# pdh930105/ARCQuant

Measured on AMD Instinct MI355X. Metric: ARC-NVFP4 GEMM TFLOP/s (M=4096, N=KQ=4096, KE=64), higher is better.
Workload: dtype f16

## Files before the change

### arcquant_amd/csrc/gemm_tile.hip

```cpp
#include <hip/hip_runtime.h>
#include <stdint.h>
#include <stdlib.h>

#include <type_traits>

#include "arcq_internal.hpp"
#include "gemm_common.hpp"
#include "gemm_tile_common.hpp"

namespace arcq {

#ifdef ARCQ_STREAM_STAMPS
static unsigned long long* g_tile_stamps = nullptr;
#ifndef ARCQ_TILE_REPACKED_UNIT
extern "C" void arcq_debug_set_tile_stamps(void* p) { g_tile_stamps = reinterpret_cast<unsigned long long*>(p); }
#endif
#define ARCQ_TILE_STAMP(k)                                                                                     \
  do {                                                                                                         \
    if (p.stamps && tid == 0) {                                                                                \
      unsigned long long t0_, t1_;                                                                             \
      asm volatile("s_memtime %0\n\ts_memrealtime %1\n\ts_waitcnt lgkmcnt(0)" : "=s"(t0_), "=s"(t1_)::"memory"); \
      p.stamps[(size_t)blockIdx.x * (2 * kTileStamps) + 2 * (k)] = t0_;                                        \
      p.stamps[(size_t)blockIdx.x * (2 * kTileStamps) + 2 * (k) + 1] = t1_;                                    \
    }                                                                                                          \
  } while (0)
#else
#define ARCQ_TILE_STAMP(k) do { } while (0)
#endif

#ifndef ARCQ_TILE_WIDE_STORES
#define ARCQ_TILE_WIDE_STORES 1
#endif

template <int BM, int BN, int WAVES_M, int WAVES_N, bool kMfma32, int kEpi, bool kStagger, bool kPipe, int kBLayout = kBRef>
__global__ __launch_bounds__(WAVES_M* WAVES_N * 64) void gemm_tile_kernel(TileParams p) {
  constexpr int kThreads = WAVES_M * WAVES_N * 64;
  constexpr int WM = BM / WAVES_M, WN = BN / WAVES_N;
  constexpr int kT = kMfma32 ? 32 : 16;
  constexpr int TM = WM / kT, TN = WN / kT;
  using acc_t = typename std::conditional<kMfma32, f32x16, f32x4>::type;
  constexpr int A_UNITS = (BM * 2 + kThreads - 1) / kThreads, B_UNITS = (BN * 2 + kThreads - 1) / kThreads;
  constexpr bool A_PARTIAL = (BM * 2) % kThreads != 0, B_PARTIAL = (BN * 2) % kThreads != 0;
  static_assert(!A_PARTIAL || A_UNITS == 1, "a partial A pass is a single pass");
  static_assert(!B_PARTIAL || B_UNITS == 1, "a partial B pass is a single pass");
  constexpr int A_TILE = BM * kRowBytes, B_TILE = BN * kRowBytes;

  extern __shared__ __attribute__((aligned(16))) unsigned char smem[];
  unsigned char* const lds_a0 = smem;
  unsigned char* const lds_b0 = smem + A_TILE;
  unsigned char* const lds_a1 = smem + A_TILE + B_TILE;
  unsigned char* const lds_b1 = smem + 2 * A_TILE + B_TILE;

  const int ntiles = p.tiles_m * p.tiles_n;
  int bid = blockIdx.x, split = 0;
  if (p.splits > 1) {
    split = bid / ntiles;
    bid -= split * ntiles;
  }
  {
    const int q8 = ntiles >> 3, r8 = ntiles & 7, x = bid & 7, j = bid >> 3;
    bid = (x < r8 ? x * (q8 + 1) : r8 * (q8 + 1) + (x - r8) * q8) + j;
  }
  constexpr int kGroupM = 8;
  const int per_group = kGroupM * p.tiles_n;
  const int grp = bid / per_group;
  const int first_m = grp * kGroupM;
  const int gsz = min(p.tiles_m - first_m, kGroupM);
  const int tm = first_m + (bid % per_group) % gsz;
  const int tn = (bid % per_group) / gsz;
  const int m0 = __builtin_amdgcn_readfirstlane(tm * BM), n0 = __builtin_amdgcn_readfirstlane(tn * BN);

  const int tid = threadIdx.x;
  const int lane = tid & 63, wave = tid >> 6;
  const int wr = wave / WAVES_N, wc = wave % WAVES_N;
  ARCQ_TILE_STAMP(0);
  const int half_k = p.K >> 1, atoms_k = p.K >> 6;
  const int a_begin = split * p.atoms_per_split, a_end = min(atoms_k, a_begin + p.atoms_per_split);

  const uint8_t* a_q[A_UNITS];
  const uint8_t* a_sf[A_UNITS];
  uint32_t a_live[A_UNITS];
  int a_slot[A_UNITS][4];
#pragma unroll
  for (int u = 0; u < A_UNITS; ++u) {
    const int unit = tid + u * kThreads, r = A_PARTIAL ? min(unit >> 1, BM - 1) : unit >> 1, h = unit & 1;
    const int row = m0 + r, rc = row < p.M ? row : p.M - 1;
    a_q[u] = p.A + (size_t)rc * half_k + h * 16;
    a_sf[u] = p.SFA + sf_atom_offset(rc, 0, atoms_k) + h * 2;
    a_live[u] = row < p.M ? 0xffffu : 0u;
#pragma unroll
    for (int j = 0; j < 4; ++j) a_slot[u][j] = kMfma32 ? lds_slot32(r, h * 4 + j) : lds_slot(r, h * 4 + j);
  }
  const uint8_t* b_q[B_UNITS];
  const uint8_t* b_sf[B_UNITS];
  uint32_t b_live[B_UNITS];
  int b_slot[B_UNITS][4];
#pragma unroll
  for (int u = 0; u < B_UNITS; ++u) {
    const int unit = tid + u * kThreads, r = B_PARTIAL ? min(unit >> 1, BN - 1) : unit >> 1, h = unit & 1;
    const int row = n0 + r, rc = row < p.N ? row : p.N - 1;
    if constexpr (kBLayout == kBRepacked) {
      const int tiles = ((p.K + 255) >> 8) * 2;
      b_q[u] = p.B + (size_t)(rc >> 4) * tiles * 1024 + h * 256 + (rc & 15) * 16;
      b_sf[u] = p.SFB + (size_t)(rc >> 4) * tiles * 128 + h * 64 + (rc & 15) * 4;
    } else {
      b_q[u] = p.B + (size_t)rc * half_k + h * 16;
      b_sf[u] = p.SFB + sf_atom_offset(rc, 0, atoms_k) + h * 2;
    }
    b_live[u] = row < p.N ? 0xffffu : 0u;
#pragma unroll
    for (int j = 0; j < 4; ++j) b_slot[u][j] = kMfma32 ? lds_slot32(r, h * 4 + j) : lds_slot(r, h * 4 + j);
  }
  const int fa_base = kMfma32 ? lds_slot32(wr * WM + (lane & 31), lane >> 5) : lds_slot(wr * WM + (lane & 15), lane >> 4);
  const int fb_base = kMfma32 ? lds_slot32(wc * WN + (lane & 31), lane >> 5) : lds_slot(wc * WN + (lane & 15), lane >> 4);
  acc_t acc[TM][TN];
#pragma unroll
  for (int i = 0; i < TM; ++i)
#pragma unroll
    for (int j = 0; j < TN; ++j)
#pragma unroll
      for (int r = 0; r < (kMfma32 ? 16 : 4); ++r) acc[i][j][r] = 0.f;

  Staged sa[A_UNITS], sb[B_UNITS];
  auto load_step = [&](int atom) {
#pragma unroll
    for (int u = 0; u < A_UNITS; ++u) sa[u] = stage_load(a_q[u], a_sf[u], atom);
#pragma unroll
    for (int u = 0; u < B_UNITS; ++u) sb[u] = kBLayout == kBRepacked ? stage_load_rw(b_q[u], b_sf[u], atom) : stage_load(b_q[u], b_sf[u], atom);
  };
  auto store_step = [&](unsigned char* la, unsigned char* lb) {
#pragma unroll
    for (int u = 0; u < A_UNITS; ++u)
      if (!A_PARTIAL || tid < BM * 2) stage_store(la, a_slot[u], sa[u], a_live[u]);
#pragma unroll
    for (int u = 0; u < B_UNITS; ++u)
      if (!B_PARTIAL || tid < BN * 2) stage_store(lb, b_slot[u], sb[u], b_live[u]);
  };
  auto mma_step = [&](const unsigned char* la, const unsigned char* lb) {
    if constexpr (kMfma32) {
#pragma unroll
      for (int ks = 0; ks < 4; ++ks) {
        Frag8 fa[TM], fb[TN];
#pragma unroll
        for (int i = 0; i < TM; ++i) fa[i].u = *reinterpret_cast<const uint4*>(la + (fa_base ^ (ks * 32)) + i * 32 * kRowBytes);
#pragma unroll
        for (int j = 0; j < TN; ++j) fb[j].u = *reinterpret_cast<const uint4*>(lb + (fb_base ^ (ks * 32)) + j * 32 * kRowBytes);
#pragma unroll
        for (int i = 0; i < TM; ++i)
#pragma unroll
          for (int j = 0; j < TN; ++j) acc[i][j] = __builtin_amdgcn_mfma_f32_32x32x16_f16(fb[j].v, fa[i].v, acc[i][j], 0, 0, 0);
      }
    } else {
#pragma unroll
      for (int ks = 0; ks < 2; ++ks) {
        Frag8 fa[TM], fb[TN];
#pragma unroll
        for (int i = 0; i < TM; ++i) fa[i].u = *reinterpret_cast<const uint4*>(la + (fa_base ^ (ks * 64)) + i * 16 * kRowBytes);
#pragma unroll
        for (int j = 0; j < TN; ++j) fb[j].u = *reinterpret_cast<const uint4*>(lb + (fb_base ^ (ks * 64)) + j * 16 * kRowBytes);
#pragma unroll
        for (int i = 0; i < TM; ++i)
#pragma unroll
          for (int j = 0; j < TN; ++j) acc[i][j] = __builtin_amdgcn_mfma_f32_16x16x32_f16(fb[j].v, fa[i].v, acc[i][j], 0, 0, 0);
      }
    }
  };
  const bool late = kStagger && wave >= 4;
  auto k_step = [&](int kt, unsigned char* ca, unsigned char* cb, unsigned char* na, unsigned char* nb) {
    Staged ta[A_UNITS], tb[B_UNITS];
#pragma unroll
    for (int u = 0; u < A_UNITS; ++u) ta[u] = sa[u];
#pragma unroll
    for (int u = 0; u < B_UNITS; ++u) tb[u] = sb[u];
    load_step(min(kt + 2 + (late ? 1 : 0), a_end - 1));
    __builtin_amdgcn_sched_barrier(0);
    mma_step(ca, cb);
    if (kStagger && late) __syncthreads();
    unsigned char* const wa = late ? ca : na;
    unsigned char* const wb = late ? cb : nb;
#pragma unroll
    for (int u = 0; u < A_UNITS; ++u)
      if (!A_PARTIAL || tid < BM * 2) stage_store(wa, a_slot[u], ta[u], a_live[u]);
#pragma unroll
    for (int u = 0; u < B_UNITS; ++u)
      if (!B_PARTIAL || tid < BN * 2) stage_store(wb, b_slot[u], tb[u], b_live[u]);
    if (!kStagger || !late) __syncthreads();
  };

  auto k_step_pipe = [&](int kt, unsigned char* ca, unsigned char* cb, unsigned char* na, unsigned char* nb) {
    static_assert(kMfma32 || TM % 2 == 0, "pairs of A fragments");
    Staged ta[A_UNITS], tb[B_UNITS];
#pragma unroll
    for (int u = 0; u < A_UNITS; ++u) ta[u] = sa[u];
#pragma unroll
    for (int u = 0; u < B_UNITS; ++u) tb[u] = sb[u];
    load_step(min(kt + 2, a_end - 1));
    __builtin_amdgcn_sched_barrier(0);
    constexpr int kPieces = (A_UNITS + B_UNITS) * 4, kBlocks = kMfma32 ? 4 : TM;
    auto pieces = [&](int blk) {
#pragma unroll
      for (int c = blk; c < kPieces; c += kBlocks) {
        const int u = c >> 2, j = c & 3;
        if (u < A_UNITS) {
#ifdef ARCQ_EXPERIMENT_A_RAW
          if (!A_PARTIAL || tid < BM * 2) stage_piece_raw(na, a_slot[u < A_UNITS ? u : 0][j], ta[u < A_UNITS ? u : 0], a_live[u < A_UNITS ? u : 0], j);
#else
          if (!A_PARTIAL || tid < BM * 2) stage_piece(na, a_slot[u < A_UNITS ? u : 0][j], ta[u < A_UNITS ? u : 0], a_live[u < A_UNITS ? u : 0], j);
#endif
        } else {
          const int v = u - A_UNITS < B_UNITS ? u - A_UNITS : 0;
#ifdef ARCQ_EXPERIMENT_B_RAW
          if (!B_PARTIAL || tid < BN * 2) stage_piece_raw(nb, b_slot[v][j], tb[v], b_live[v], j);
#else
          if (!B_PARTIAL || tid < BN * 2) stage_piece(nb, b_slot[v][j], tb[v], b_live[v], j);
#endif
        }
      }
    };
    if constexpr (kMfma32) {
      Frag8 f32a[2][TM], f32b[2][TN];
      auto rd_set = [&](int buf, int ks) {
#pragma unroll
        for (int i = 0; i < TM; ++i) f32a[buf][i].u = *reinterpret_cast<const uint4*>(ca + (fa_base ^ (ks * 32)) + i * 32 * kRowBytes);
#pragma unroll
        for (int j = 0; j < TN; ++j) f32b[buf][j].u = *reinterpret_cast<const uint4*>(cb + (fb_base ^ (ks * 32)) + j * 32 * kRowBytes);
      };
      rd_set(0, 0);
#pragma unroll
      for (int ks = 0; ks < 4; ++ks) {
        if (ks + 1 < 4) rd_set((ks + 1) & 1, ks + 1);
        __builtin_amdgcn_sched_barrier(0);
#pragma unroll
        for (int i = 0; i < TM; ++i)
#pragma unroll
          for (int j = 0; j < TN; ++j)
            if constexpr (kMfma32)
              acc[i][j] = __builtin_amdgcn_mfma_f32_32x32x16_f16(f32b[ks & 1][j].v, f32a[ks & 1][i].v, acc[i][j], 0, 0, 0);
        pieces(ks);
        __builtin_amdgcn_sched_barrier(0);
      }
      __syncthreads();
      return;
    }
    auto rd_a = [&](int ks, int i) { Frag8 f; f.u = *reinterpret_cast<const uint4*>(ca + (fa_base ^ (ks * 64)) + i * 16 * kRowBytes); return f; };
    auto rd_b = [&](int ks, int j) { Frag8 f; f.u = *reinterpret_cast<const uint4*>(cb + (fb_base ^ (ks * 64)) + j * 16 * kRowBytes); return f; };
    constexpr int kPairs = TM / 2, kSeq = 2 * kPairs, kAhead = 1;
    Frag8 fb[2][TN], fq[kSeq][2];
    auto rd_pair = [&](int q) {
      fq[q][0] = rd_a(q / kPairs, 2 * (q % kPairs));
      fq[q][1] = rd_a(q / kPairs, 2 * (q % kPairs) + 1);
    };
#pragma unroll
    for (int j = 0; j < TN; ++j) fb[0][j] = rd_b(0, j);
#pragma unroll
    for (int q = 0; q < kAhead; ++q) rd_pair(q);
#pragma unroll
    for (int q = 0; q < kSeq; ++q) {
      const int ks = q / kPairs, pr = q % kPairs;
      if (q + kAhead < kSeq) rd_pair(q + kAhead);
      if (ks == 0 && pr == kPairs - 1 - (kAhead - 1 < kPairs - 1 ? kAhead - 1 : kPairs - 1)) {
#pragma unroll
        for (int j = 0; j < TN; ++j) fb[1][j] = rd_b(1, j);
      }
      __builtin_amdgcn_sched_barrier(0);
#pragma unroll
      for (int ii = 0; ii < 2; ++ii)
#pragma unroll
        for (int j = 0; j < TN; ++j)
          if constexpr (!kMfma32)
            acc[2 * pr + ii][j] = __builtin_amdgcn_mfma_f32_16x16x32_f16(fb[ks][j].v, fq[q][ii].v, acc[2 * pr + ii][j], 0, 0, 0);
      pieces(q);
#pragma unroll
      for (int m8 = 0; m8 < (TM == 8 ? 2 * TN : 0); ++m8) {
        __builtin_amdgcn_sched_group_barrier(0x008, 1, 0);
        __builtin_amdgcn_sched_group_barrier(0x002, 2, 0);
      }
      __builtin_amdgcn_sched_barrier(0);
    }
    __syncthreads();
  };

  load_step(a_begin);
  Staged sa0[A_UNITS], sb0[B_UNITS];
#pragma unroll
  for (int u = 0; u < A_UNITS; ++u) sa0[u] = sa[u];
#pragma unroll
  for (int u = 0; u < B_UNITS; ++u) sb0[u] = sb[u];
  load_step(min(a_begin + 1, a_end - 1));
  __builtin_amdgcn_sched_barrier(0);
#pragma unroll
  for (int u = 0; u < A_UNITS; ++u)
    if (!A_PARTIAL || tid < BM * 2) stage_store(lds_a0, a_slot[u], sa0[u], a_live[u]);
#pragma unroll
  for (int u = 0; u < B_UNITS; ++u)
    if (!B_PARTIAL || tid < BN * 2) stage_store(lds_b0, b_slot[u], sb0[u], b_live[u]);
  if (kStagger && late) {
    store_step(lds_a1, lds_b1);
    load_step(min(a_begin + 2, a_end - 1));
  }
  __syncthreads();
  int kt = a_begin;
#ifndef ARCQ_EXPERIMENT_GENERAL_EPILOGUE
  float alpha_dev = 1.0f;
  if (p.alpha_dev) alpha_dev = *reinterpret_cast<const __attribute__((address_space(4))) float*>(reinterpret_cast<uintptr_t>(p.alpha_dev));
  asm volatile("" : "+s"(alpha_dev));
#endif
  if (WAVES_M * WAVES_N == 8 && wave >= 4) __builtin_amdgcn_s_setprio(1);
  ARCQ_TILE_STAMP(1);
  if constexpr (kPipe) {
    for (; kt + 1 < a_end; kt += 2) {
      k_step_pipe(kt, lds_a0, lds_b0, lds_a1, lds_b1);
      k_step_pipe(kt + 1, lds_a1, lds_b1, lds_a0, lds_b0);
    }
    if (kt < a_end) k_step_pipe(kt, lds_a0, lds_b0, lds_a1, lds_b1);
  } else {
    for (; kt + 1 < a_end; kt += 2) {
      k_step(kt, lds_a0, lds_b0, lds_a1, lds_b1);
      k_step(kt + 1, lds_a1, lds_b1, lds_a0, lds_b0);
    }
    if (kt < a_end) k_step(kt, lds_a0, lds_b0, lds_a1, lds_b1);
  }
  ARCQ_TILE_STAMP(2);

#ifdef ARCQ_EXPERIMENT_GENERAL_EPILOGUE
  const float alpha = p.alpha_host * (p.alpha_dev ? *p.alpha_dev : 1.0f);
#else
  const float alpha = p.alpha_host * alpha_dev;
#endif
  const bool vec_ok = (p.N & 3) == 0;
  uint32_t act_max = 0;
  [[maybe_unused]] auto interior_epilogue = [&](auto has_bias, auto has_res) __attribute__((always_inline)) {
    constexpr bool kBias = decltype(has_bias)::value, kRes = decltype(has_res)::value;
    constexpr bool kSilu = kEpi == kEpiSiluMul;
    constexpr uint32_t kElem = kSilu ? 1 : 2;
    unsigned char* const tile_d = reinterpret_cast<unsigned char*>(p.D) + ((size_t)m0 * p.N + n0) * kElem;
    const unsigned char* const tile_r = kRes ? reinterpret_cast<const unsigned char*>(p.residual) + ((size_t)m0 * p.N + n0) * 2 : nullptr;
    uint32_t t = tid;
    asm volatile("" : "+v"(t));
    const uint32_t lane_row = (t >> 6) / WAVES_N * WM + (t & 15), lane_col = (t >> 6) % WAVES_N * WN + 4 * ((t >> 4) & 3);
    uint32_t off = lane_row * (uint32_t)p.N + lane_col;
    const uint32_t row_step = 16u * (uint32_t)p.N;
    constexpr bool kWide = ARCQ_TILE_WIDE_STORES && !kSilu && TN % 2 == 0;
    typedef uint32_t u32x4_a8 __attribute__((ext_vector_type(4), aligned(8)));
    [[maybe_unused]] const uint32_t g4 = (t >> 4) & 3;
    [[maybe_unused]] uint32_t off_w = off - 4 * g4 + ((g4 & 1) ? 16 + 4 * (g4 - 1) : 4 * g4);
    [[maybe_unused]] uint2 held = make_uint2(0, 0);
    float bias_f[TN][4];
    if constexpr (kBias) {
#pragma unroll
      for (int j = 0; j < TN; ++j) {
        const uint2 b = *reinterpret_cast<const uint2*>(p.bias + n0 + lane_col + j * 16);
        bias_f[j][0] = bf16_bits_to_f32(b.x & 0xffffu); bias_f[j][1] = bf16_bits_to_f32(b.x >> 16);
        bias_f[j][2] = bf16_bits_to_f32(b.y & 0xffffu); bias_f[j][3] = bf16_bits_to_f32(b.y >> 16);
      }
    }
    uint2 res_cur[TN], res_nxt[TN];
    auto res_load = [&](uint32_t o, uint2 (&r)[TN]) {
#pragma unroll
      for (int j = 0; j < TN; ++j) r[j] = *reinterpret_cast<const uint2*>(tile_r + (size_t)o * 2 + j * 32);
    };
    if constexpr (kRes) res_load(off, res_cur);
#pragma unroll
    for (int i = 0; i < TM; ++i) {
      if constexpr (kRes) { if (i + 1 < TM) res_load(off + row_step, res_nxt); }
#pragma unroll
      for (int j = 0; j < TN; ++j) {
        float d[4] = {alpha * acc[i][j][0], alpha * acc[i][j][1], alpha * acc[i][j][2], alpha * acc[i][j][3]};
        if constexpr (kSilu) {
          if constexpr (kBias) {
#pragma unroll
            for (int r = 0; r < 4; r += 2) {
              round2_to_bf16(d[r], d[r + 1]);
              d[r] += bias_f[j][r];
              d[r + 1] += bias_f[j][r + 1];
            }
          }
          const uint32_t y01 = pack_bf16x2_hw(d[0], d[1]), y23 = pack_bf16x2_hw(d[2], d[3]);
          const uint32_t a0 = silu_mul_bf16(y01 & 0xffffu, y01 >> 16), a1 = silu_mul_bf16(y23 & 0xffffu, y23 >> 16);
          *reinterpret_cast<uint32_t*>(tile_d + (size_t)off + j * 16) = a0 | (a1 << 16);
          act_max = max(act_max, max(a0 & 0x7fffu, a1 & 0x7fffu));
        } else {
          if constexpr (kBias) {
#pragma unroll
            for (int r = 0; r < 4; r += 2) {
              round2_to_bf16(d[r], d[r + 1]);
              d[r] += bias_f[j][r];
              d[r + 1] += bias_f[j][r + 1];
            }
          }
          if constexpr (kRes) {
            const uint32_t rw[2] = {res_cur[j].x, res_cur[j].y};
#pragma unroll
            for (int r = 0; r < 4; r += 2) {
              round2_to_bf16(d[r], d[r + 1]);
              d[r] += bf16_bits_to_f32(rw[r >> 1] & 0xffffu);
              d[r + 1] += bf16_bits_to_f32(rw[r >> 1] >> 16);
            }
          }
          const uint2 pk = make_uint2(pack_bf16x2_hw(d[0], d[1]), pack_bf16x2_hw(d[2], d[3]));
          if constexpr (kWide) {
            if (j & 1) {
              const auto lo = __builtin_amdgcn_permlane16_swap(held.x, pk.x, false, false);
              const auto hi = __builtin_amdgcn_permlane16_swap(held.y, pk.y, false, false);
              const u32x4_a8 v = {lo[0], hi[0], lo[1], hi[1]};
              *reinterpret_cast<u32x4_a8*>(tile_d + (size_t)off_w * 2 + (j >> 1) * 64) = v;
            } else {
              held = pk;
            }
          } else {
            *reinterpret_cast<uint2*>(tile_d + (size_t)off * 2 + j * 32) = pk;
          }
        }
        if (i == 0 && j == 0) ARCQ_TILE_STAMP(3);
      }
      if constexpr (kRes) {
#pragma unroll
        for (int j = 0; j < TN; ++j) res_cur[j] = res_nxt[j];
      }
      off += row_step;
      off_w += row_step;
    }
  };
  auto store4 = [&](int m, int n, float d0, float d1, float d2, float d3, bool pre, uint2 bias2, uint2 res2) __attribute__((always_inline)) {
    if (m >= p.M || n >= p.N) return;
    const uint32_t bw[2] = {bias2.x, bias2.y}, rw[2] = {res2.x, res2.y};
    auto bias_at = [&](int r) { return bf16_bits_to_f32(pre ? (bw[r >> 1] >> (16 * (r & 1))) & 0xffffu : (uint32_t)p.bias[n + r]); };
    if (kEpi == kEpiSiluMul) {
      uint32_t y[4] = {f32_to_bf16_bits(alpha * d0), f32_to_bf16_bits(alpha * d1), f32_to_bf16_bits(alpha * d2), f32_to_bf16_bits(alpha * d3)};
      if (p.bias) {
#pragma unroll
        for (int e = 0; e < 4; ++e) y[e] = f32_to_bf16_bits(bf16_bits_to_f32(y[e]) + bias_at(e));
      }
      const uint32_t a0 = silu_mul_bf16(y[0], y[1]);
      const uint32_t a1 = silu_mul_bf16(y[2], y[3]);
      *reinterpret_cast<uint32_t*>(reinterpret_cast<uint16_t*>(p.D) + (size_t)m * (p.N >> 1) + (n >> 1)) = a0 | (a1 << 16);
      act_max = max(act_max, max(a0 & 0x7fffu, a1 & 0x7fffu));
      return;
    }
    if (p.splits > 1) {
      *reinterpret_cast<float4*>(p.partial + ((size_t)split * p.M + m) * p.N + n) = make_float4(d0, d1, d2, d3);
      return;
    }
    float d[4] = {alpha * d0, alpha * d1, alpha * d2, alpha * d3};
    if (p.bias) {
#pragma unroll
      for (int r = 0; r < 4; ++r)
        if (pre || n + r < p.N) d[r] = (p.out_dtype == ARCQ_OUT_F32 ? d[r] : bf16_bits_to_f32(f32_to_bf16_bits(d[r]))) + bias_at(r);
    }
    if (p.residual) {
#pragma unroll
      for (int r = 0; r < 4; ++r)
        if (pre || n + r < p.N) {
          const float res = bf16_bits_to_f32(pre ? (rw[r >> 1] >> (16 * (r & 1))) & 0xffffu : (uint32_t)p.residual[(size_t)m * p.N + n + r]);
          d[r] = (p.out_dtype == ARCQ_OUT_F32 ? d[r] : bf16_bits_to_f32(f32_to_bf16_bits(d[r]))) + res;
        }
    }
    if (p.out_dtype == ARCQ_OUT_F32) {
      float* o = reinterpret_cast<float*>(p.D) + (size_t)m * p.N + n;
      if (vec_ok) *reinterpret_cast<float4*>(o) = make_float4(d[0], d[1], d[2], d[3]);
      else for (int r = 0; r < 4; ++r) if (n + r < p.N) o[r] = d[r];
    } else {
      uint16_t* o = reinterpret_cast<uint16_t*>(p.D) + (size_t)m * p.N + n;
      if (vec_ok) *reinterpret_cast<uint2*>(o) = make_uint2(pack_bf16x2(d[0], d[1]), pack_bf16x2(d[2], d[3]));
      else for (int r = 0; r < 4; ++r) if (n + r < p.N) o[r] = (uint16_t)f32_to_bf16_bits(d[r]);
    }
  };
#ifdef ARCQ_EXPERIMENT_GENERAL_EPILOGUE
  constexpr bool kInteriorPath = false;
#else
  constexpr bool kInteriorPath = !kMfma32;
#endif
  bool interior = false;
  if constexpr (kInteriorPath)
    interior = m0 + BM <= p.M && n0 + BN <= p.N && vec_ok && p.splits <= 1 && p.out_dtype == ARCQ_OUT_BF16 && (int64_t)BM * p.N < (1ll << 31) &&
               ((reinterpret_cast<uintptr_t>(p.bias) | reinterpret_cast<uintptr_t>(p.residual)) & 7) == 0;
  if (interior) {
    if constexpr (kInteriorPath) {
      using T = std::true_type;
      using F = std::false_type;
      if constexpr (kEpi == kEpiSiluMul) {
        if (p.bias) interior_epilogue(T{}, F{});
        else interior_epilogue(F{}, F{});
      } else if (p.bias) {
        if (p.residual) interior_epilogue(T{}, T{});
        else interior_epilogue(T{}, F{});
      } else {
        if (p.residual) interior_epilogue(F{}, T{});
        else interior_epilogue(F{}, F{});
      }
    }
  } else if constexpr (kMfma32) {
#pragma unroll
    for (int i = 0; i < TM; ++i)
#pragma unroll
      for (int j = 0; j < TN; ++j) {
        const int m = m0 + wr * WM + i * 32 + (lane & 31);
#pragma unroll
        for (int g = 0; g < 4; ++g) {
          const int n = n0 + wc * WN + j * 32 + 8 * g + 4 * (lane >> 5);
          store4(m, n, acc[i][j][4 * g + 0], acc[i][j][4 * g + 1], acc[i][j][4 * g + 2], acc[i][j][4 * g + 3], false, make_uint2(0, 0), make_uint2(0, 0));
        }
      }
  } else {
    const bool pre = vec_ok && p.splits <= 1 && ((reinterpret_cast<uintptr_t>(p.bias) | reinterpret_cast<uintptr_t>(p.residual)) & 7) == 0;
    const int nb = n0 + wc * WN + 4 * (lane >> 4), mb = m0 + wr * WM + (lane & 15);
    if (pre) {
      uint2 bias_v[TN], res_cur[TN], res_nxt[TN];
#pragma unroll
      for (int j = 0; j < TN; ++j) {
        bias_v[j] = res_cur[j] = res_nxt[j] = make_uint2(0, 0);
        if (p.bias && nb + j * 16 < p.N) bias_v[j] = *reinterpret_cast<const uint2*>(p.bias + nb + j * 16);
      }
      auto res_load = [&](int i, uint2 (&r)[TN]) {
        if (!p.residual) return;
        const int m = mb + i * 16;
#pragma unroll
        for (int j = 0; j < TN; ++j)
          if (m < p.M && nb + j * 16 < p.N) r[j] = *reinterpret_cast<const uint2*>(p.residual + (size_t)m * p.N + nb + j * 16);
      };
      res_load(0, res_cur);
#pragma unroll
      for (int i = 0; i < TM; ++i) {
        if (i + 1 < TM) res_load(i + 1, res_nxt);
#pragma unroll
        for (int j = 0; j < TN; ++j) {
          store4(mb + i * 16, nb + j * 16, acc[i][j][0], acc[i][j][1], acc[i][j][2], acc[i][j][3], true, bias_v[j], res_cur[j]);
          if (i == 0 && j == 0) ARCQ_TILE_STAMP(3);
        }
#pragma unroll
        for (int j = 0; j < TN; ++j) res_cur[j] = res_nxt[j];
      }
    } else {
#pragma unroll
      for (int i = 0; i < TM; ++i)
#pragma unroll
        for (int j = 0; j < TN; ++j) {
          store4(mb + i * 16, nb + j * 16, acc[i][j][0], acc[i][j][1], acc[i][j][2], acc[i][j][3], false, make_uint2(0, 0), make_uint2(0, 0));
          if (i == 0 && j == 0) ARCQ_TILE_STAMP(3);
        }
    }
  }
  ARCQ_TILE_STAMP(4);
  if (kEpi == kEpiSiluMul) {
    __shared__ uint32_t wave_max[WAVES_M * WAVES_N];
#pragma unroll
    for (int sh = 32; sh > 0; sh >>= 1) act_max = max(act_max, (uint32_t)__shfl_down((int)act_max, sh, 64));
    if (lane == 0) wave_max[wave] = act_max;
    __syncthreads();
    if (tid == 0) {
      uint32_t m = 0;
#pragma unroll
      for (int w = 0; w < WAVES_M * WAVES_N; ++w) m = max(m, wave_max[w]);
      p.slots[blockIdx.x] = m;
    }
  }
}

struct TileCfg { int id, bm, bn, waves; };
static constexpr TileCfg kTileCfgs[] = {{1, 128, 128, 4}, {2, 256, 256, 4}, {3, 256, 256, 8}, {4, 128, 256, 4}, {5, 256, 256, 8}, {6, 128, 128, 4},
                                        {7, 64, 256, 4}, {8, 32, 256, 4}, {9, 128, 128, 4}, {10, 128, 256, 8}, {11, 256, 128, 8}, {12, 128, 128, 8},
                                        {13, 64, 256, 8}, {14, 64, 128, 8}, {15, 64, 64, 4}, {16, 64, 128, 4}, {17, 128, 64, 4}};
static const TileCfg& tile_cfg(int id) {
  for (const TileCfg& c : kTileCfgs)
    if (c.id == id) return c;
  return kTileCfgs[2];
}

static int env_int(const char* name, int dflt) {
  const char* e = getenv(name);
  return e ? atoi(e) : dflt;
}
static int tile_cfg_override() {
  static const int v = env_int("ARCQ_TILE_CFG", 0);
  return v;
}
static int tile_split_override() {
  static const int v = env_int("ARCQ_TILE_SPLIT", 0);
  return v;
}
static bool tile_stagger() {
  static const int v = env_int("ARCQ_TILE_STAGGER", 0);
  return v != 0;
}
static bool tile_pipe() {
  static const int v = env_int("ARCQ_TILE_PIPE", 1);
  return v != 0;
}

static void tile_split(int64_t M, int64_t N, int64_t K, int BM, int BN, int* splits, int* atoms_per_split) {
  const int64_t tiles = ((M + BM - 1) / BM) * ((N + BN - 1) / BN);
  const int atoms = (int)(K / 64);
  int s = 1;
  if ((N % 4) == 0) {
    if (tile_split_override() > 0) s = min(tile_split_override(), max(atoms / 2, 1));
    else
      while (tiles * s < 256 && atoms / (s * 2) >= 8 && s < 32) s *= 2;
  }
  const int per = (atoms + s - 1) / s;
  *splits = (atoms + per - 1) / per;
  *atoms_per_split = per;
}

template <int BM, int BN, int WAVES_M, int WAVES_N, bool kMfma32 = false, int kEpi = kEpiPlain, int kBLayout = kBRef>
static int launch_tile(const GemmArgs& a, hipStream_t stream, bool allow_split = false) {
  TileParams p;
  p.A = a.A; p.B = a.B; p.SFA = a.SFA; p.SFB = a.SFB; p.D = a.D;
  p.alpha_dev = a.alpha_dev; p.bias = a.bias; p.residual = a.residual;
  p.M = a.M; p.N = a.N; p.K = a.K; p.alpha_host = a.alpha_host; p.out_dtype = a.out_dtype;
  p.tiles_m = (a.M + BM - 1) / BM;
  p.tiles_n = (a.N + BN - 1) / BN;
  p.splits = 1; p.atoms_per_split = a.K / 64; p.partial = nullptr;
  p.epi = a.epilogue; p.slots = a.absmax_slots;
#ifdef ARCQ_STREAM_STAMPS
  p.stamps = g_tile_stamps;
#endif
  if (allow_split && a.epilogue == kEpiPlain) {
    tile_split(a.M, a.N, a.K, BM, BN, &p.splits, &p.atoms_per_split);
    if (p.splits > 1) {
      const int64_t need = (int64_t)p.splits * a.M * a.N * (int64_t)sizeof(float);
      if (!a.workspace || a.workspace_bytes < need)
        return fail(ARCQ_ERR_WORKSPACE, "arcq_gemm_nvfp4: split-K needs %lld B of workspace, got %lld", (long long)need,
                    (long long)a.workspace_bytes);
      p.partial = reinterpret_cast<float*>(a.workspace);
    }
  }
  const size_t lds = 2 * (size_t)(BM + BN) * kRowBytes;
  constexpr bool kCanStagger = WAVES_M * WAVES_N == 8 && BM == 256 && BN == 256, kCanPipe = true;
  auto kern = gemm_tile_kernel<BM, BN, WAVES_M, WAVES_N, kMfma32, kEpi, false, false, kBLayout>;
  if (kCanPipe && tile_pipe()) kern = gemm_tile_kernel<BM, BN, WAVES_M, WAVES_N, kMfma32, kEpi, false, kCanPipe, kBLayout>;
  else if (kCanStagger && tile_stagger()) kern = gemm_tile_kernel<BM, BN, WAVES_M, WAVES_N, kMfma32, kEpi, kCanStagger, false, kBLayout>;
  static LdsOptIn lds_opt[3];
  const int which = (kCanPipe && tile_pipe()) ? 1 : (kCanStagger && tile_stagger()) ? 2 : 0;
  if (int rc = ensure_dynamic_lds(reinterpret_cast<const void*>(kern), lds_opt[which], (int)lds, "arcq_gemm_nvfp4 (tile)")) return rc;
  hipLaunchKernelGGL(kern, dim3((unsigned)(p.tiles_m * p.tiles_n * p.splits)), dim3(WAVES_M * WAVES_N * 64), lds, stream, p);
  hipError_t e = hipGetLastError();
  if (e != hipSuccess) return fail(ARCQ_ERR_LAUNCH, "arcq_gemm_nvfp4 (tile): launch failed: %s", hipGetErrorString(e));
  if (p.splits > 1) return gemm_splitk_finish(a, p.splits, stream);
  return ARCQ_OK;
}

static int tile_choice(int64_t M, int64_t N, int64_t K) {
  const int64_t t256 = ((M + 255) / 256) * ((N + 255) / 256);
  if (t256 >= 192) return 3;
  if (M <= 32) return 8;
  if (M <= 64) return 7;
  const int64_t t10 = ((M + 127) / 128) * ((N + 255) / 256);
  if (t10 <= 64 || t10 == 128 || (t10 > 224 && t10 <= 256) || (K >= 8192 && t10 >= 96 && t10 <= 256)) return 10;
  return 1;
}

static int effective_cfg(int64_t M, int64_t N, int64_t K, bool* may_split) {
  int id = tile_cfg_override();
  if (id == 0) id = tile_choice(M, N, K);
  id = tile_cfg(id).id;
  *may_split = !(id >= 2 && id <= 6) && id != 9;
  return id;
}

#ifndef ARCQ_TILE_REPACKED_UNIT
int64_t gemm_tile_silu_slots(int64_t M, int64_t N, int64_t K) {
  bool sp;
  const TileCfg& c = tile_cfg(effective_cfg(M, N, K, &sp));
  return ((M + c.bm - 1) / c.bm) * ((N + c.bn - 1) / c.bn);
}

int64_t gemm_tile_workspace_bytes(int64_t M, int64_t N, int64_t K) {
  int s = 1, per = 0;
  bool sp;
  const TileCfg& c = tile_cfg(effective_cfg(M, N, K, &sp));
  if (sp) tile_split(M, N, K, c.bm, c.bn, &s, &per);
  return s > 1 ? (int64_t)s * M * N * (int64_t)sizeof(float) : 0;
}
#endif

template <int kEpi, int kBLayout>
static int gemm_tile_epi(const GemmArgs& a, hipStream_t stream) {
  bool sp;
  switch (effective_cfg(a.M, a.N, a.K, &sp)) {
    case 1: case 9: return launch_tile<128, 128, 2, 2, false, kEpi, kBLayout>(a, stream, sp);
    case 2: return launch_tile<256, 256, 2, 2, false, kEpi, kBLayout>(a, stream);
    case 4: return launch_tile<128, 256, 2, 2, false, kEpi, kBLayout>(a, stream);
    case 5: return launch_tile<256, 256, 2, 4, true, kEpi, kBLayout>(a, stream);
    case 6: return launch_tile<128, 128, 2, 2, true, kEpi, kBLayout>(a, stream);
    case 7: return launch_tile<64, 256, 1, 4, false, kEpi, kBLayout>(a, stream, sp);
    case 8: return launch_tile<32, 256, 1, 4, false, kEpi, kBLayout>(a, stream, sp);
    case 10: return launch_tile<128, 256, 2, 4, false, kEpi, kBLayout>(a, stream, sp);
    case 11: return launch_tile<256, 128, 4, 2, false, kEpi, kBLayout>(a, stream, sp);
    case 12: return launch_tile<128, 128, 2, 4, false, kEpi, kBLayout>(a, stream, sp);
    case 13: return launch_tile<64, 256, 1, 8, false, kEpi, kBLayout>(a, stream, sp);
    case 14: return launch_tile<64, 128, 2, 4, false, kEpi, kBLayout>(a, stream, sp);
    case 15: return launch_tile<64, 64, 2, 2, false, kEpi, kBLayout>(a, stream, sp);
    case 16: return launch_tile<64, 128, 2, 2, false, kEpi, kBLayout>(a, stream, sp);
    case 17: return launch_tile<128, 64, 2, 2, false, kEpi, kBLayout>(a, stream, sp);
    default: return launch_tile<256, 256, 2, 4, false, kEpi, kBLayout>(a, stream);
  }
}

#ifndef ARCQ_TILE_REPACKED_UNIT
int gemm_tile(const GemmArgs& a, hipStream_t stream) {
  if (a.b_layout == kBRepacked) return gemm_tile_repacked(a, stream);
  return a.epilogue == kEpiSiluMul ? gemm_tile_epi<kEpiSiluMul, kBRef>(a, stream) : gemm_tile_epi<kEpiPlain, kBRef>(a, stream);
}
#else
int gemm_tile_repacked(const GemmArgs& a, hipStream_t stream) {
  return a.epilogue == kEpiSiluMul ? gemm_tile_epi<kEpiSiluMul, kBRepacked>(a, stream) : gemm_tile_epi<kEpiPlain, kBRepacked>(a, stream);
}
#endif

}
```

Before: 1442.

## Rotate k-step pipeline so the barrier sits before the final MFMA blocks

```diff
diff --git a/arcquant_amd/csrc/gemm_tile.hip b/arcquant_amd/csrc/gemm_tile.hip
--- a/arcquant_amd/csrc/gemm_tile.hip
+++ b/arcquant_amd/csrc/gemm_tile.hip
@@ -30,6 +30,13 @@
 
 #ifndef ARCQ_TILE_WIDE_STORES
 #define ARCQ_TILE_WIDE_STORES 1
+#endif
+
+#ifndef ARCQ_TILE_BARRIER_AT_STEP_END
+#define ARCQ_TILE_BARRIER_AT_STEP_END 0
+#endif
+#ifndef ARCQ_TILE_ROT
+#define ARCQ_TILE_ROT 1
 #endif
 
 template <int BM, int BN, int WAVES_M, int WAVES_N, bool kMfma32, int kEpi, bool kStagger, bool kPipe, int kBLayout = kBRef>
@@ -187,6 +194,10 @@
     if (!kStagger || !late) __syncthreads();
   };
 
+  constexpr int kRot = ARCQ_TILE_ROT;
+  constexpr bool kRotate = !ARCQ_TILE_BARRIER_AT_STEP_END && kPipe && !kMfma32 && TM == 8 && TN == 4 && WAVES_M * WAVES_N == 8 && !A_PARTIAL && !B_PARTIAL;
+  auto rd_frag = [&](const unsigned char* tile, int base, int ks, int i) { Frag8 f; f.u = *reinterpret_cast<const uint4*>(tile + (base ^ (ks * 64)) + i * 16 * kRowBytes); return f; };
+  [[maybe_unused]] Frag8 head_b[TN], head_a[2];
   auto k_step_pipe = [&](int kt, unsigned char* ca, unsigned char* cb, unsigned char* na, unsigned char* nb) {
     static_assert(kMfma32 || TM % 2 == 0, "pairs of A fragments");
     Staged ta[A_UNITS], tb[B_UNITS];
@@ -242,8 +253,77 @@
       __syncthreads();
       return;
     }
-    auto rd_a = [&](int ks, int i) { Frag8 f; f.u = *reinterpret_cast<const uint4*>(ca + (fa_base ^ (ks * 64)) + i * 16 * kRowBytes); return f; };
-    auto rd_b = [&](int ks, int j) { Frag8 f; f.u = *reinterpret_cast<const uint4*>(cb + (fb_base ^ (ks * 64)) + j * 16 * kRowBytes); return f; };
+    auto rd_a = [&](int ks, int i) { return rd_frag(ca, fa_base, ks, i); };
+    auto rd_b = [&](int ks, int j) { return rd_frag(cb, fb_base, ks, j); };
+    if constexpr (kRotate) {
+      constexpr int kQ = 2 * (TM / 2), kHalf = TM / 2, kLast = kQ - 1 - kRot, kNPre = kLast + 1;
+      static_assert(kRot >= 1 && kLast >= kHalf, "the second K half's B fragments are read ahead of the barrier, a block before their use");
+      auto read_by = [](int b) { const int extra = b - (kLast - kRot), h = b + 1 + (extra > 0 ? extra : 0); return h < kQ - 1 ? h : kQ - 1; };
+      Frag8 fb1[TN], fq[kQ][2];
+      fq[0][0] = head_a[0];
+      fq[0][1] = head_a[1];
+#pragma unroll
+      for (int q = 0; q < kQ; ++q) {
+        const int ks = q / kHalf, pr = q % kHalf;
+        constexpr int kHeadReads = TN + 2;
+        int n_pieces = 0, n_reads = 0;
+        if (q <= kLast) {
+#pragma unroll
+          for (int r = (q ? read_by(q - 1) : 0) + 1; r <= read_by(q); ++r) {
+            fq[r][0] = rd_a(r / kHalf, 2 * (r % kHalf));
+            fq[r][1] = rd_a(r / kHalf, 2 * (r % kHalf) + 1);
+          }
+          if (q == kHalf - 1) {
+#pragma unroll
+            for (int j = 0; j < TN; ++j) fb1[j] = rd_b(1, j);
+          }
+        }
+        __builtin_amdgcn_sched_barrier(0);
+#pragma unroll
+        for (int ii = 0; ii < 2; ++ii)
+#pragma unroll
+          for (int j = 0; j < TN; ++j)
+            acc[2 * pr + ii][j] = __builtin_amdgcn_mfma_f32_16x16x32_f16((ks ? fb1[j] : head_b[j]).v, fq[q][ii].v, acc[2 * pr + ii][j], 0, 0, 0);
+        if (q <= kLast) {
+#pragma unroll
+          for (int c = 0; c < kPieces; ++c)
+            if (c * kNPre / kPieces == q) {
+              const int u = c >> 2, j = c & 3;
+              if (u < A_UNITS) {
+                stage_piece(na, a_slot[u][j], ta[u], a_live[u], j);
+              } else {
+                stage_piece(nb, b_slot[u - A_UNITS][j], tb[u - A_UNITS], b_live[u - A_UNITS], j);
+              }
+              ++n_pieces;
+            }
+        } else {
+          const int i0 = q - kLast - 1;
+#pragma unroll
+          for (int n = i0 * kHeadReads / kRot; n < (i0 + 1) * kHeadReads / kRot; ++n) {
+            if (n < TN) head_b[n] = rd_frag(nb, fb_base, 0, n);
+            else head_a[n - TN] = rd_frag(na, fa_base, 0, n - TN);
+            ++n_reads;
+          }
+        }
+#pragma unroll
+        for (int m8 = 0; m8 < 2 * TN; ++m8) {
+          __builtin_amdgcn_sched_group_barrier(0x008, 1, 0);
+          if (q <= kLast) {
+            if (n_pieces == 1) __builtin_amdgcn_sched_group_barrier(0x002, 2, 0);
+            else if (n_pieces == 2) __builtin_amdgcn_sched_group_barrier(0x002, 4, 0);
+            else if (n_pieces >= 3) __builtin_amdgcn_sched_group_barrier(0x002, 6, 0);
+          } else if (m8 < n_reads) {
+            __builtin_amdgcn_sched_group_barrier(0x100, 1, 0);
+          }
+        }
+        __builtin_amdgcn_sched_barrier(0);
+        if (q == kLast) {
+          __syncthreads();
+          __builtin_amdgcn_sched_barrier(0);
+        }
+      }
+      return;
+    }
     constexpr int kPairs = TM / 2, kSeq = 2 * kPairs, kAhead = 1;
     Frag8 fb[2][TN], fq[kSeq][2];
     auto rd_pair = [&](int q) {
@@ -299,6 +379,12 @@
     load_step(min(a_begin + 2, a_end - 1));
   }
   __syncthreads();
+  if constexpr (kRotate) {
+#pragma unroll
+    for (int j = 0; j < TN; ++j) head_b[j] = rd_frag(lds_b0, fb_base, 0, j);
+    head_a[0] = rd_frag(lds_a0, fa_base, 0, 0);
+    head_a[1] = rd_frag(lds_a0, fa_base, 0, 1);
+  }
   int kt = a_begin;
 #ifndef ARCQ_EXPERIMENT_GENERAL_EPILOGUE
   float alpha_dev = 1.0f;
```

After: 1459 (median of 6 runs). 1.01x the previous value.
